# dark-Stallion/alac

Measured on AMD Instinct MI355X. Metric: encode Msamples/s (bit-exact) 44.1kHz/16-bit stereo, 1/2/4/8 GPU, higher is better.
Workload: dtype int32 (int16 PCM, int16 coefficients)

## Files before the change

### alac_amd/csrc/alac_encode_v1_impl.hpp

```cpp
#pragma once
#include <cstdlib>
#include <type_traits>
#include "alac_encode_v1_types.hpp"
#include "alac_lms.hpp"
#include "alac_golomb.hpp"

namespace alacdev {

template <int N, int I = 0, class F>
__device__ __forceinline__ void static_for(F &&f)
{
    if constexpr (I < N) {
        f(std::integral_constant<int, I>{});
        static_for<N, I + 1>(f);
    }
}

constexpr int kHist = 12;
template <int LPC>
struct Geo {
    static constexpr int TILE = LPC == 1 ? 32 : 64;
    static constexpr int ROWLEN = kHist + TILE;
    static constexpr int STRIDE = ROWLEN + 9;
};
// ... 266 lines not shown
        P.xs[it] = row * Geo<LPC>::STRIDE + kHist + grp * 4;
        const int32_t r = CH == 2 ? sh.rowMix[row] : 0;
        P.wl[it] = r ? r : (1 << kMixBits);
        P.wr[it] = r ? (1 << kMixBits) - r : 0;
        P.vsel[it] = r ? -1 : 0;
    }
}

template <int DEPTH, int CH, int LPC>
__device__ __forceinline__ void stage_load_fast(StageRegs<CH, LPC> &R, const StagePlan<CH, LPC> &P, int j0)
{
    constexpr int BPF = CH * (int)bytes_per_sample(DEPTH);
    const int64_t byteOff = (int64_t)j0 * BPF;
#pragma unroll
    for (int it = 0; it < StagePlan<CH, LPC>::ITERS; it++) task_load<DEPTH, CH>(P.pk[it] + byteOff, R.v[it]);
}

template <int LPC, bool HEAD = false>
__device__ __forceinline__ void keep_history(LmsShared<LPC> &sh, int lane)
{
    constexpr int SLOTS = 64 / LPC, N = kHist * SLOTS / 64;
    static_assert(kHist * SLOTS % 64 == 0, "every lane moves the same number of cells");
    int32_t v[N];
#pragma unroll
    for (int it = 0; it < N; it++) {
        const int idx = it * 64 + lane, row = idx % SLOTS, c = idx / SLOTS;
        v[it] = HEAD ? 0 : sh.xs[row * Geo<LPC>::STRIDE + Geo<LPC>::TILE + c];
    }
#pragma unroll
    for (int it = 0; it < N; it++) {
        const int idx = it * 64 + lane, row = idx % SLOTS, c = idx / SLOTS;
        sh.xs[row * Geo<LPC>::STRIDE + c] = v[it];
    }
}

template <int DEPTH, int CH, int LPC>
__device__ __forceinline__ void stage_store_fast(const StageRegs<CH, LPC> &R, const StagePlan<CH, LPC> &P,
                                                 LmsShared<LPC> &sh)
{
#pragma unroll
    for (int it = 0; it < StagePlan<CH, LPC>::ITERS; it++) {
        static_for<4>([&](auto T) {
            constexpr int t = decltype(T)::value;
            if constexpr (CH == 2) {
                const int32_t l = task_sample<DEPTH, 2 * t>(R.v[it]), r = task_sample<DEPTH, 2 * t + 1>(R.v[it]);
                sh.xs[P.xs[it] + t] = (__mul24(P.wl[it], l) + __mul24(P.wr[it], r)) >> kMixBits;
                sh.xs[P.xs[it] + Geo<LPC>::STRIDE + t] = P.vsel[it] ? l - r : r;
            } else {
                sh.xs[P.xs[it] + t] = task_sample<DEPTH, t>(R.v[it]);
            }
        });
    }
}

struct StepOps {
    int32_t nx[8], tp[8], cu[8];
};

__device__ __forceinline__ void load_ops(StepOps &o, const int32_t *pn, const int32_t *pt, const int32_t *pc)
{
#pragma unroll
    for (int s = 0; s < 8; s++) {
        o.nx[s] = pn[s];
        o.tp[s] = pt[s];
        o.cu[s] = pc[s];
    }
}

template <int T, int LPC, bool MASKED, bool DEAD = (T > 4)>
__device__ __forceinline__ void run_block(int32_t (&a)[T], int32_t (&w)[T], const StepOps &o, const LmsLaneT<T> &L, int jb,
                                          int32_t *resAt, uint32_t chanbits)
{
#pragma unroll
    for (int s = 0; s < 8; s++) {
        const int j = jb + s;
        const int32_t liveMask = MASKED ? (((j >= L.jlo) & (j < L.jhi)) ? -1 : 0) : -1;
        resAt[s] = lms_step<T, LPC, MASKED, DEAD>(a, w, o.tp[s], o.cu[s], liveMask, L, chanbits);
#pragma unroll
        for (int i = T - 1; i > 0; i--) w[i] = w[i - 1];
        w[0] = o.nx[s];
    }
}

struct LaneView {
    const int32_t *row;
    int32_t *res;
    const int32_t *zero;
    bool feeds;
};

template <int T, int LPC, bool DEAD = (T > 4)>
__device__ __forceinline__ void run_tile(int32_t (&a)[T], const LaneView &V, const LmsLaneT<T> &L, int j0, int jEnd,
                                         uint32_t chanbits)
{
    const int adv = V.feeds ? 1 : 0;
    const int32_t *pn = V.feeds ? V.row + kHist - T * L.h : V.zero;
    const int32_t *pt = V.feeds ? V.row + kHist - 1 - L.na : V.zero;
    const int32_t *pc = V.row + kHist;
    int32_t w[T];
#pragma unroll
    for (int i = 0; i < T; i++) w[i] = V.feeds ? V.row[kHist - 1 - T * L.h - i] : 0;
    StepOps opA, opB;
    load_ops(opA, pn, pt, pc);
    auto block = [&](const StepOps &cur, StepOps &nxt, int jb) {
        const int o = jb - j0;
        load_ops(nxt, pn + adv * (o + 8), pt + adv * (o + 8), pc + (o + 8));
        const bool allLive = __all((jb >= L.jlo) & (jb + 8 <= L.jhi));
        if (allLive)
            run_block<T, LPC, false, DEAD>(a, w, cur, L, jb, V.res + o, chanbits);
        else
            run_block<T, LPC, true, DEAD>(a, w, cur, L, jb, V.res + o, chanbits);
    };
    for (int jb = j0; jb < jEnd; jb += 16) {
        block(opA, opB, jb);
        if (jb + 8 < jEnd) block(opB, opA, jb + 8);
        else opA = opB;
    }
}

struct ChainJob {
    bool active;
    uint32_t seg, ch, p, N;
    int na;
    int16_t *row;
};

struct NoSink {};
template <int DEPTH, int CH, int LPC, bool WT = false, bool ZZ = false, int T = 4, class Sink = NoSink, bool DEAD = (T > 4)>
__device__ __forceinline__ void lms_pass(LmsShared<LPC> &sh, const V1Args &A, const ChainJob &J, int32_t (&a)[T],
                                         uint32_t num, uint32_t P, bool store, int32_t *dst, uint64_t streamStride,
                                         uint32_t stream, int lane, uint32_t *flag = nullptr, uint32_t flagBase = 0,
                                         StageRegs<CH, LPC> *head = nullptr, int headMode = 0, Sink *sink = nullptr)
{
    constexpr int SLOTS = 64 / LPC;
    constexpr uint32_t chanBits = DEPTH - 8 * bytes_shifted(DEPTH) + (CH == 2 ? 1 : 0);
    const uint32_t frameBytes = A.S.frameSize * CH * bytes_per_sample(DEPTH);
    const int slot = lane / LPC;
    LmsLaneT<T> L = make_lane<T, LPC>(lane, J.na, J.active ? (int)num : 0);
    const uint32_t idleVal = A.idleFast ? 0xffffffffu : 0u;
    if (!J.active && A.idleFast) {
        L.jlo = 0;
        L.jhi = 0x7fffffff;
    }
    LaneView V;
    V.feeds = J.active && (T * L.h < J.na);
    V.row = sh.xs + slot * Geo<LPC>::STRIDE;
    V.res = V.feeds ? sh.xs + slot * Geo<LPC>::STRIDE : sh.xs + SLOTS * Geo<LPC>::STRIDE;
    V.zero = sh.zero;
    const int fs = lane % SLOTS;
    const uint32_t fP = (uint32_t)__shfl((int)(J.active ? P : 0), fs * LPC);
    const uint32_t fStream = (uint32_t)__shfl((int)stream, fs * LPC);
    const int fNa = __shfl(J.na, fs * LPC);
    const uint32_t runTo = wave_max(J.active ? (store ? (P > num ? P : num) : num) : 0);
    const uint32_t half = (uint32_t)(lane / SLOTS);
    const uint32_t voff = half * (uint32_t)streamStride + fStream;
    const bool fAct = __shfl((int)J.active, fs * LPC) != 0;
    const uint32_t fPmin = wave_min_u32(fAct ? fP : idleVal);
    StageRegs<CH, LPC> R;
    StagePlan<CH, LPC> SP;
    stage_plan<DEPTH, CH, LPC>(SP, sh, A.S.pcm, frameBytes, lane);
    const uint32_t nMinRows = wave_min_u32(J.active ? J.N : idleVal);
    auto interior = [&](int j) { return SP.usable && (uint32_t)(j + Geo<LPC>::TILE) <= nMinRows; };
    if (runTo > 0) {
        if (interior(0)) {
            keep_history<LPC, true>(sh, lane);
            if (head && headMode == 2) {
                stage_store_fast<DEPTH, CH, LPC>(*head, SP, sh);
            } else {
                stage_load_fast<DEPTH, CH, LPC>(R, SP, 0);
                if (head && headMode == 1) {
                    constexpr int BPF = CH * (int)bytes_per_sample(DEPTH);
#pragma unroll
                    for (int it = 0; it < StagePlan<CH, LPC>::ITERS; it++)
#pragma unroll
                        for (int k = 0; k <= BPF; k++) head->v[it][k] = R.v[it][k];
                }
                stage_store_fast<DEPTH, CH, LPC>(R, SP, sh);
            }
        } else {
            stage_load<DEPTH, CH, LPC>(R, sh, A.S.pcm, frameBytes, 0, lane);
            stage_store<DEPTH, CH, LPC>(R, sh, A.S.pcm, frameBytes, 0, lane);
        }
    }
    for (int j0 = 0; j0 < (int)runTo; j0 += Geo<LPC>::TILE) {
        const bool more = j0 + Geo<LPC>::TILE < (int)runTo;
        const bool fastNext = more && interior(j0 + Geo<LPC>::TILE);
        if (fastNext) stage_load_fast<DEPTH, CH, LPC>(R, SP, j0 + Geo<LPC>::TILE);
        else if (more) stage_load<DEPTH, CH, LPC>(R, sh, A.S.pcm, frameBytes, j0 + Geo<LPC>::TILE, lane);
        lds_order();
        if (store && j0 == 0) {
            for (int pos = lane / SLOTS; pos <= fNa; pos += LPC) {
                const int32_t *xr = sh.xs + fs * Geo<LPC>::STRIDE + kHist;
                sh.xs[fs * Geo<LPC>::STRIDE + Geo<LPC>::ROWLEN + pos] = pos == 0 ? xr[0] : sext(xr[pos] - xr[pos - 1], 32 - chanBits);
            }
            lds_order();
        }
        const int jEnd = min(j0 + Geo<LPC>::TILE, (int)((runTo + 7) & ~7u));
        run_tile<T, LPC, DEAD>(a, V, L, j0, jEnd, chanBits);
        lds_order();
        if (store) {
            if (j0 == 0) {
                for (int pos = lane / SLOTS; pos <= fNa; pos += LPC)
                    sh.xs[fs * Geo<LPC>::STRIDE + pos] = sh.xs[fs * Geo<LPC>::STRIDE + Geo<LPC>::ROWLEN + pos];
                lds_order();
            }
            using Cell = int32_t __attribute__((ext_vector_type(4)));
            auto put4 = [&](const char *rowBase, uint32_t off, const int32_t *v) {
                auto zz = [](int32_t x) { return ZZ ? (int32_t)(((uint32_t)x << 1) ^ (uint32_t)(x >> 31)) : x; };
                Cell c;
                c.x = zz(v[0]);
                c.y = zz(v[1]);
                c.z = zz(v[2]);
                c.w = zz(v[3]);
                if constexpr (WT)
                    asm volatile("global_store_dwordx4 %0, %1, %2 sc1\n\ts_nop 1" : : "v"(off), "v"(c), "s"(rowBase) : "memory");
                else
                    *(Cell *)(rowBase + off) = c;
            };
            if constexpr (!std::is_same<Sink, NoSink>::value) {
                static_assert(LPC == 1, "a tile sink reads the lane's own row");
                (*sink)(j0, sh.xs + fs * Geo<LPC>::STRIDE);
            }
            constexpr int CELLS = Geo<LPC>::TILE / 4 / LPC;
            const int32_t *cell = sh.xs + fs * Geo<LPC>::STRIDE + 4 * (int)half;
            const char *rowPtr = dst ? (const char *)(dst + (uint64_t)j0 * streamStride) : nullptr;
            const uint64_t rowStep = (uint64_t)LPC * streamStride * 16u;
            const uint32_t laneOff = voff * 16u;
            if (!std::is_same<Sink, NoSink>::value && !dst) {
            } else if constexpr (LPC >= 2) {
                if ((uint32_t)(j0 + Geo<LPC>::TILE) <= fPmin) {
                    int32_t v[CELLS][4];
#pragma unroll
                    for (int it = 0; it < CELLS; it++)
#pragma unroll
                        for (int k = 0; k < 4; k++) v[it][k] = cell[it * 4 * LPC + k];
                    lds_order();
                    uint32_t off = laneOff;
                    asm volatile("" : "+v"(off));
#pragma unroll
                    for (int it = 0; it < CELLS; it++) {
                        put4(rowPtr, off, v[it]);
                        rowPtr += rowStep;
                    }
                } else {
                    constexpr int GROUP = 2;
                    static_assert(CELLS % GROUP == 0, "whole groups");
#pragma unroll 1
                    for (int g = 0; g < CELLS; g += GROUP) {
                        int32_t v[GROUP][4];
#pragma unroll
                        for (int k = 0; k < GROUP; k++)
#pragma unroll
                            for (int e = 0; e < 4; e++) v[k][e] = cell[(g + k) * 4 * LPC + e];
                        lds_order();
#pragma unroll
                        for (int k = 0; k < GROUP; k++) {
                            const uint32_t j = (uint32_t)(j0 + 4 * ((g + k) * LPC + (int)half));
                            if (j < fP) put4(rowPtr, laneOff, v[k]);
                            rowPtr += rowStep;
                        }
                        lds_order();
                    }
                }
            } else {
                const bool whole = (uint32_t)(j0 + Geo<LPC>::TILE) <= fPmin;
#pragma unroll
                for (int it = 0; it < CELLS; it++) {
                    int32_t v[4];
#pragma unroll
                    for (int k = 0; k < 4; k++) v[k] = cell[it * 4 + k];
                    if (whole || (uint32_t)(j0 + 4 * it) < fP) put4(rowPtr, laneOff, v);
                    rowPtr += rowStep;
                }
            }
            if (flag) {
                const uint32_t pm = A.pubMask & 0xffu;
                const uint32_t tile = (uint32_t)j0 / (uint32_t)Geo<LPC>::TILE;
                if ((tile & pm) == pm || (uint32_t)j0 + (pm + 1) * (uint32_t)Geo<LPC>::TILE >= runTo)
                    publish_rows(flag, flagBase + (uint32_t)min(j0 + Geo<LPC>::TILE, (int)runTo), lane, (A.pubMask >> 31) != 0, A.ho.lose);
            }
        }
// ... 3 lines not shown
            lds_order();
            stage_store_fast<DEPTH, CH, LPC>(R, SP, sh);
        } else if (more) {
            stage_store<DEPTH, CH, LPC>(R, sh, A.S.pcm, frameBytes, j0 + Geo<LPC>::TILE, lane);
        }
    }
}

template <int LPC>
__device__ __forceinline__ void lms_setup(LmsShared<LPC> &sh, const ChainJob &J, int mix, int lane)
{
    constexpr int SLOTS = 64 / LPC;
    if (lane < kZeroCells) sh.zero[lane] = 0;
    if (lane % LPC == 0) {
        const int slot = lane / LPC;
        sh.pktIdx[slot] = J.p;
        sh.pktN[slot] = J.active ? J.N : 0;
        sh.rowMix[slot] = mix;
    }
    (void)SLOTS;
    lds_order();
}

template <int LPC, int T = 4>
__device__ __forceinline__ void load_row(const ChainJob &J, int32_t (&a)[T], int lane, bool virgin = false)
{
    const int h = lane & (LPC - 1);
#pragma unroll
    for (int i = 0; i < T; i++) {
        const int k = T * h + i;
        const int32_t init = k == 0 ? 1216 : (k == 1 ? -928 : (k == 2 ? -64 : 0));
        a[i] = (J.active && k < J.na) ? (virgin ? init : (int32_t)J.row[k]) : 0;
    }
}

__device__ __forceinline__ int pick_mixres(const V1Args &A, uint32_t seg)
{
    uint32_t best = 0, minb = 1u << 31;
#pragma unroll
    for (uint32_t r = 0; r <= (uint32_t)kMaxRes; r++) {
        const uint32_t tot = A.bits1[r * A.chainsPad + seg * 2] + A.bits1[r * A.chainsPad + seg * 2 + 1];
        if (tot < minb) {
            minb = tot;
            best = r;
        }
    }
    return (int)best;
}

struct PacketDecision {
    uint32_t num[2];
    uint32_t escape;
};
template <int DEPTH, int CH>
__device__ __forceinline__ PacketDecision decide_packet(const V1Args &A, uint32_t seg, uint32_t N)
{
    constexpr uint32_t SHB = bytes_shifted(DEPTH);
    PacketDecision D;
    D.num[1] = 0;
    uint32_t minBits = 0;
#pragma unroll
    for (uint32_t c = 0; c < (uint32_t)CH; c++) {
        const uint32_t chain = seg * CH + c;
        const uint32_t c4 = A.cost2[chain], c8 = A.cost2[A.chainsPad + chain];
        D.num[c] = c8 < c4 ? 8 : 4;
        minBits += c8 < c4 ? c8 : c4;
    }
    const uint32_t partial = (N != A.S.frameSize);
    minBits += (CH == 2 ? 64 : 32) + (partial ? 32 : 0) + N * (SHB * 8) * CH;
    const uint32_t escapeBits = N * DEPTH * CH + (partial ? 32 : 0) + 16;
    D.escape = minBits >= escapeBits ? 1u : 0u;
    return D;
}

template <int LPC, int T = 4>
__device__ __forceinline__ void store_row(const ChainJob &J, const int32_t (&a)[T], int lane)
{
    const int h = lane & (LPC - 1);
#pragma unroll
    for (int i = 0; i < T; i++)
        if (J.active && T * h + i < J.na) J.row[T * h + i] = (int16_t)a[i];
}

template <int DEPTH, int T, int L>
__device__ __forceinline__ void search1_predictor(LmsShared<L> &sh, const V1Args &A, uint32_t block, int lane, uint32_t *flag)
{
    constexpr int SLOTS = 64 / L;
    ChainJob J;
    const uint32_t chain = A.S.segBegin * 2 + block * SLOTS + lane / L;
    J.seg = chain >> 1;
    J.ch = chain & 1;
    J.active = seg_packet(A.S, J.seg, J.p, J.N);
    J.na = 8;
    J.row = A.state + (uint64_t)J.seg * 64 + J.ch * 32 + 16;
    if (A.rowReady && A.S.pos > 0) {
        bool wait = false;
        if (J.active) {
            const PacketRec *prev = A.recs + (J.p - 1);
            wait = !prev->escape && prev->c[J.ch].num == 8;
        }
        bool seen = false;
        for (uint32_t spins = 0; spins < A.ho.spinLimit; spins++) {
            const uint32_t r = wait ? __hip_atomic_load(A.rowReady + chain, __ATOMIC_RELAXED, __HIP_MEMORY_SCOPE_AGENT) : 0xffffffffu;
            if (__all(r >= A.S.pos)) {
                seen = true;
                break;
            }
            __builtin_amdgcn_s_sleep(16);
        }
        if (!seen && A.ho.err && lane == 0) __hip_atomic_store(A.ho.err, 1u, __ATOMIC_RELAXED, __HIP_MEMORY_SCOPE_SYSTEM);
        __builtin_amdgcn_fence(__ATOMIC_ACQUIRE, "agent");
    }
    int32_t a[T];
    load_row<L>(J, a, lane, A.virgin != 0);
    const uint32_t n8 = J.N / 8;
    constexpr bool keepHead = L != 1;
    StageRegs<2, L> headRegs;
    StageRegs<2, L> *head = keepHead ? &headRegs : nullptr;
    for (int r = 0; r <= kMaxRes; r++) {
        lms_setup<L>(sh, J, r, lane);
        if (flag)
            lms_pass<DEPTH, 2, L, true>(sh, A, J, a, n8, n8, true, A.resA, 5ull * A.chainsPad, (uint32_t)r * A.chainsPad + chain,
                                        lane, flag, (uint32_t)r << 16, head, r == 0 ? 1 : 2);
        else
            lms_pass<DEPTH, 2, L>(sh, A, J, a, n8, n8, true, A.resA, 5ull * A.chainsPad, (uint32_t)r * A.chainsPad + chain, lane,
                                  nullptr, 0, head, r == 0 ? 1 : 2);
    }
    store_row<L>(J, a, lane);
    if (flag) publish_rows(flag, 0xffffffffu, lane, (A.pubMask >> 31) != 0, A.ho.lose);
}

template <int DEPTH, int T, int L>
__global__ __launch_bounds__(64, L == 1 ? 2 : 1) void k_lms_search1(V1Args A)
{
    __shared__ LmsShared<L> sh;
    search1_predictor<DEPTH, T, L>(sh, A, blockIdx.x, threadIdx.x, nullptr);
}

template <int DEPTH, int CH, int RS, int T, int LPC>
__device__ __forceinline__ void search2_body(LmsShared<LPC> &sh, const V1Args &A, uint32_t block, int lane)
{
    constexpr int SLOTS = 64 / LPC;
    constexpr int rs = RS;
    ChainJob J;
    const uint32_t chain = A.S.segBegin * CH + block * SLOTS + lane / LPC;
    J.seg = chain / CH;
    J.ch = chain % CH;
    J.active = seg_packet(A.S, J.seg, J.p, J.N);
    J.na = rs ? 8 : 4;
    J.row = A.state + (uint64_t)J.seg * 64 + J.ch * 32 + rs * 16;
    int32_t a[T];
    load_row<LPC>(J, a, lane, A.virgin != 0 && (rs == 0 || CH == 1));
    const int best = (CH == 2 && J.active) ? pick_mixres(A, J.seg) : 0;
    if (CH == 2 && rs == 1 && J.active && J.ch == 0 && (lane % LPC) == 0) A.recs[J.p].mixRes = (uint32_t)best;
    lms_setup<LPC>(sh, J, best, lane);
    const uint32_t n8 = J.N / 8, n32 = J.N / 32;
    StageRegs<CH, LPC> head;
    for (int pass = 0; pass < 8; pass++) {
        const bool last = pass == 7;
        const uint32_t num = (CH == 1 && last) ? n8 : n32;
        uint32_t P = num > (uint32_t)(J.na + 1) ? num : (uint32_t)(J.na + 1);
        P = P < n8 ? P : n8;
        lms_pass<DEPTH, CH, LPC>(sh, A, J, a, num, P, last, A.resB, 2ull * A.chainsPad, (uint32_t)rs * A.chainsPad + chain,
                                 lane, nullptr, 0, &head, pass == 0 ? 1 : 2);
    }
    store_row<LPC>(J, a, lane);
}

template <int DEPTH, int CH, int T3 = 4, int L3 = 1, int T7 = 4, int L7 = 2, int WAVES = 1>
__global__ __launch_bounds__(64, WAVES) void k_lms_search2(V1Args A, uint32_t nb3)
{
    __shared__ union {
        LmsShared<L3> s1;
        LmsShared<L7> s2;
    } sh;
    if (blockIdx.x < nb3)
        search2_body<DEPTH, CH, 0, T3, L3>(sh.s1, A, blockIdx.x, threadIdx.x);
    else
        search2_body<DEPTH, CH, 1, T7, L7>(sh.s2, A, blockIdx.x - nb3, threadIdx.x);
}

template <int DEPTH, int CH>
__global__ __launch_bounds__(64 * kWavesPerWg, 1) void k_lms_search2_w(V1Args A, uint32_t nb3, uint32_t nb7)
{
    __shared__ union {
        LmsShared<1> s1;
        LmsShared<2> s2;
    } shAll[kWavesPerWg];
    const Worker W = worker_id();
    auto &sh = shAll[W.slot];
    const uint32_t t = W.id / 3, r = W.id % 3;
    if (r == 0) {
        if (t < nb3) search2_body<DEPTH, CH, 0, 4, 1>(sh.s1, A, t, W.lane);
    } else {
        const uint32_t b = 2 * t + r - 1;
        if (b < nb7) search2_body<DEPTH, CH, 1, 4, 2>(sh.s2, A, b, W.lane);
    }
}

template <int DEPTH, int CH>
__global__ __launch_bounds__(64) void k_lms_final(V1Args A)
{
    __shared__ LmsShared<2> sh;
    const int lane = threadIdx.x;
    ChainJob J;
    const uint32_t chain = A.S.segBegin * CH + blockIdx.x * 32u + lane / 2;
    J.seg = chain / CH;
    J.ch = chain % CH;
    J.active = seg_packet(A.S, J.seg, J.p, J.N);
    J.na = 4;
    int best = 0;
    uint32_t N = J.N;
    if (J.active) {
        const PacketRec *rec = A.recs + J.p;
        J.na = rec->c[J.ch].num;
        best = (int)rec->mixRes;
        if (rec->escape) {
            J.active = false;
        }
    }
    J.row = A.state + (uint64_t)J.seg * 64 + J.ch * 32 + (J.na == 8 ? 16 : 0);
    int32_t a[4];
    load_row<2>(J, a, lane);
    lms_setup<2>(sh, J, best, lane);
    lms_pass<DEPTH, CH, 2, false, true>(sh, A, J, a, N, N, true, A.resC, A.chainsPad, chain, lane);
    store_row<2>(J, a, lane);
}


template <int CH>
__global__ __launch_bounds__(64) void k_gol_count1(V1Args A, uint32_t chanBits)
{
    __shared__ uint32_t recip[17];
    gol_table_init(recip, threadIdx.x);
    __syncthreads();
    const uint32_t chain = A.S.segBegin * CH + blockIdx.x * 64u + threadIdx.x, r = blockIdx.y;
    const uint32_t t = r * A.chainsPad + chain;
    uint32_t p, N;
    const bool active = seg_packet(A.S, chain / CH, p, N);
    const uint32_t n8 = active ? N / 8 : 0;
    const int32_t *plane = plane_from_stream(A.resA, (uint64_t)r * A.chainsPad);
    const uint64_t stride = 5ull * A.chainsPad;
    GolF g;
    golf_reset(g);
    golf_stream<false>(g, n8, wave_max(n8), chanBits, recip, one_plane(plane, stride, chain));
    if (active) A.bits1[t] = n8 ? g.bits : 0u;
}

template <int DEPTH, int T, int L, bool WALK = false>
__global__ __launch_bounds__(64 * kWavesPerWg, 1) void k_search1_fused(V1Args A, uint32_t nLms, uint32_t cblocks, uint32_t chanBits)
{
    __shared__ LmsShared<L> shAll[kWavesPerWg];
    __shared__ uint32_t recipAll[kWavesPerWg][20];
    const Worker W = worker_id();
    LmsShared<L> &sh = shAll[W.slot];
    uint32_t *recip = recipAll[W.slot];
    const int lane = W.lane;
    if constexpr (WALK) {
        if (W.id >= (uint32_t)(L + 1) * cblocks) return;
        const uint32_t t = W.id / (L + 1), r0 = W.id % (L + 1);
        if (r0 < (uint32_t)L) {
            const uint32_t pw = (uint32_t)L * t + r0;
            if (pw < nLms) search1_predictor<DEPTH, T, L>(sh, A, pw, lane, A.flags + pw);
            return;
        }
        gol_table_init(recip, lane);
        lds_order();
        const uint32_t w = t;
        const uint32_t chain = A.S.segBegin * 2 + w * 64u + lane;
        uint32_t p, N;
        const bool active = seg_packet(A.S, chain >> 1, p, N);
        const uint32_t n8 = active ? N / 8 : 0;
        const uint64_t stride = 5ull * A.chainsPad;
        RowWait wait;
        wait.producers(A.flags, L * w, L, nLms);
        wait.avail = 0;
        wait.ho = A.ho;
        const uint32_t nMax = wave_max(n8);
#pragma unroll 1
        for (uint32_t r = 0; r <= (uint32_t)kMaxRes; r++) {
            GolF g;
            golf_reset(g);
            wait.base = r << 16;
            golf_stream<false>(g, n8, nMax, chanBits, recip, one_plane(plane_from_stream(A.resA, (uint64_t)r * A.chainsPad), stride, chain), wait);
            if (active) A.bits1[r * A.chainsPad + chain] = n8 ? g.bits : 0u;
        }
        return;
    }
    if (W.id >= nLms + 5 * cblocks) return;
    if (W.id < nLms) {
        search1_predictor<DEPTH, T, L>(sh, A, W.id, lane, A.flags + W.id);
    } else {
        gol_table_init(recip, lane);
        lds_order();
        const uint32_t idx = W.id - nLms, r = idx / cblocks, w = idx % cblocks;
        const uint32_t chain = A.S.segBegin * 2 + w * 64u + lane;
        const uint32_t t = r * A.chainsPad + chain;
        uint32_t p, N;
        const bool active = seg_packet(A.S, chain >> 1, p, N);
        const uint32_t n8 = active ? N / 8 : 0;
        const int32_t *plane = plane_from_stream(A.resA, (uint64_t)r * A.chainsPad);
        const uint64_t stride = 5ull * A.chainsPad;
        GolF g;
        golf_reset(g);
        RowWait wait;
        wait.producers(A.flags, L * w, L, nLms);
        wait.avail = 0;
        wait.base = r << 16;
        wait.ho = A.ho;
        golf_stream<false>(g, n8, wave_max(n8), chanBits, recip, one_plane(plane, stride, chain), wait);
        if (active) A.bits1[t] = n8 ? g.bits : 0u;
    }
}

template <int CH, class Need>
__device__ __forceinline__ void count2_body(const V1Args &A, uint32_t chain, uint32_t rs, uint32_t chanBits, const uint32_t *recip,
                                            Need &&need)
{
    const uint32_t t = rs * A.chainsPad + chain;
    uint32_t p, N;
    const bool active = seg_packet(A.S, chain / CH, p, N);
    const uint32_t n8 = active ? N / 8 : 0, n32 = N / 32, na = rs ? 8 : 4;
    uint32_t P2 = n8;
    if (CH == 2) {
        P2 = n32 > na + 1 ? n32 : na + 1;
        P2 = P2 < n8 ? P2 : n8;
    }
    const uint64_t strideB = 2ull * A.chainsPad, strideA = 5ull * A.chainsPad;
    GolF g;
    golf_reset(g);
    const int32_t *planeB = plane_from_stream(A.resB, (uint64_t)rs * A.chainsPad), *planeA = plane_from_stream(A.resA, (uint64_t)kMaxRes * A.chainsPad);
    const uint32_t nMax = wave_max(n8);
    const uint32_t p2lo = wave_min_u32(active ? P2 : 0xffffffffu), p2hi = wave_max(active ? P2 : 0u);
    if (CH == 1 || p2lo >= p2hi) {
        RowSrc rs2;
        rs2.p0 = planeB;
        rs2.s0 = strideB;
        rs2.p1 = planeA;
        rs2.s1 = strideA;
        rs2.split = CH == 1 ? 0xffffffffu : p2hi;
        rs2.col = chain;
        rs2.org = 0;
        golf_stream<false>(g, n8, nMax, chanBits, recip, rs2, need);
    } else {
        golf_stream_fn<false>(g, n8, nMax, chanBits, recip, [&](uint32_t j) {
            const int32_t b = planeB[plane_index(j, strideB, chain)], a = planeA[plane_index(j, strideA, chain)];
            return j < P2 ? b : a;
        }, need);
    }
    if (active) A.cost2[t] = (n8 ? g.bits : 0u) * 8 + 16 * na;
}

template <int CH>
__global__ __launch_bounds__(64) void k_gol_count2(V1Args A, uint32_t chanBits)
{
    __shared__ uint32_t recip[17];
    gol_table_init(recip, threadIdx.x);
    __syncthreads();
    count2_body<CH>(A, A.S.segBegin * CH + blockIdx.x * 64u + threadIdx.x, blockIdx.y, chanBits, recip, NoWait());
}

template <int CH>
__global__ __launch_bounds__(64 * kWavesPerWg, 1) void k_gol_count2_w(V1Args A, uint32_t cblocks, uint32_t chanBits)
{
    __shared__ uint32_t recipAll[kWavesPerWg][20];
    const Worker W = worker_id();
    if (W.id >= 2 * cblocks) return;
    uint32_t *recip = recipAll[W.slot];
    gol_table_init(recip, W.lane);
    lds_order();
    count2_body<CH>(A, A.S.segBegin * CH + (W.id % cblocks) * 64u + (uint32_t)W.lane, W.id / cblocks, chanBits, recip, NoWait());
}

#ifdef ALAC_V1_COMMON_TU
// ... 78 lines not shown
    __shared__ LmsShared<L> shAll[kWavesPerWg];
    __shared__ uint32_t recipAll[kWavesPerWg][20];
    const Worker W = worker_id();
    if (W.id >= nWorkers) return;
    LmsShared<L> &sh = shAll[W.slot];
    uint32_t *recip = recipAll[W.slot];
    const int lane = W.lane;
    uint32_t wid = W.id;
    if constexpr (!SPLIT) {
        const uint32_t t = W.id / (L + 1), r = W.id % (L + 1);
        wid = r < (uint32_t)L ? (uint32_t)L * t + r : nLms + t;
        if (r < (uint32_t)L && wid >= nLms) return;
    }
    struct WaveStamp {
        uint32_t *p;
        __device__ __forceinline__ WaveStamp(uint32_t *dbg, int lane) : p(dbg ? dbg + 8ull * (blockIdx.x * (uint32_t)kWavesPerWg + (threadIdx.x >> 6)) : nullptr)
        {
            if (p && lane == 0) {
                const uint64_t t = __builtin_amdgcn_s_memtime();
                p[0] = __builtin_amdgcn_s_getreg((31 << 11) | 4);
                p[1] = __builtin_amdgcn_s_getreg((31 << 11) | 20);
                p[2] = (uint32_t)t;
                p[3] = (uint32_t)(t >> 32);
            }
        }
        __device__ __forceinline__ void done(int lane)
        {
            if (p && lane == 0) {
                const uint64_t t = __builtin_amdgcn_s_memtime();
                p[4] = (uint32_t)t;
                p[5] = (uint32_t)(t >> 32);
                p[6] = __builtin_amdgcn_s_getreg((31 << 11) | 4);
            }
        }
    } stamp(A.dbg, lane);
    if (wid < nLms) {
        ChainJob J;
        const uint32_t chain = A.S.segBegin * CH + wid * (64u / L) + lane / L;
        J.seg = chain / CH;
        J.ch = chain % CH;
        J.active = seg_packet(A.S, J.seg, J.p, J.N);
        J.na = 4;
        int best = 0;
        const uint32_t N = J.N;
        const bool have = J.active;
        if (J.active) {
            if constexpr (FOLD) {
                const PacketDecision D = decide_packet<DEPTH, CH>(A, J.seg, N);
                J.na = (int)D.num[J.ch];
                best = CH == 2 ? (int)A.recs[J.p].mixRes : 0;
                if (D.escape) J.active = false;
            } else {
                const PacketRec *rec = A.recs + J.p;
                J.na = rec->c[J.ch].num;
                best = (int)rec->mixRes;
                if (rec->escape) J.active = false;
            }
        }
        J.row = A.state + (uint64_t)J.seg * 64 + J.ch * 32 + (J.na == 8 ? 16 : 0);
        int32_t a[T];
        load_row<L>(J, a, lane);
        if constexpr (FOLD) {
            if (have) {
                PacketRec *rec = A.recs + J.p;
                const int h = lane & (L - 1);
#pragma unroll
                for (int i = 0; i < T; i++)
                    if (T * h + i < 8) rec->c[J.ch].coefs[T * h + i] = (T * h + i < J.na) ? (int16_t)a[i] : (int16_t)0;
                if (h == 0) {
                    rec->c[J.ch].num = (uint16_t)J.na;
                    if (J.ch == 0) {
                        rec->numSamples = N;
                        if (CH == 1) {
                            rec->c[1].num = 0;
                            rec->c[1].bits = 0;
                            rec->mixRes = 0;
                        }
                    }
                }
            }
        }
        lms_setup<L>(sh, J, best, lane);
        uint32_t *flag = A.flagsF + wid;
        lms_pass<DEPTH, CH, L, true, true>(sh, A, J, a, N, N, true, A.resC, A.chainsPad, chain, lane, flag);
        store_row<L>(J, a, lane);
        if (A.rowReady) {
            asm volatile("s_waitcnt vmcnt(0)" ::: "memory");
            __builtin_amdgcn_fence(__ATOMIC_RELEASE, "agent");
            asm volatile("s_waitcnt vmcnt(0)" ::: "memory");
            if (J.active && J.na == 8 && lane % L == 0 && !A.ho.lose)
                __hip_atomic_store(A.rowReady + chain, A.S.pos + 1, __ATOMIC_RELAXED, __HIP_MEMORY_SCOPE_AGENT);
        }
        publish_rows(flag, 0xffffffffu, lane, (A.pubMask >> 31) != 0, A.ho.lose);
        stamp.done(lane);
    } else {
        gol_table_init(recip, lane);
        lds_order();
        const uint32_t cb = wid - nLms;
        const bool second = SPLIT && cb >= nCoder;
        const uint32_t w = second ? cb - nCoder : cb;
        const uint32_t chain = A.S.segBegin * CH + w * 64u + lane;
        uint32_t p, N;
        bool active = seg_packet(A.S, chain / CH, p, N);
        const bool have = active;
        PacketRec *rec = A.recs + p;
        PacketDecision D;
        D.num[0] = D.num[1] = D.escape = 0;
        if constexpr (FOLD) {
            if (have) D = decide_packet<DEPTH, CH>(A, chain / CH, N);
            if (D.escape) active = false;
        } else {
            if (active && rec->escape) active = false;
        }
        const uint32_t c = chain % CH;
        const uint32_t n = active ? N : 0;
        const int32_t *plane = A.resC;
        const uint64_t stride = A.chainsPad;
        GolF g;
        golf_reset(g);
        const uint64_t slotIdx = have ? (uint64_t)p * 2 + c : (uint64_t)A.dumpSlot + c;
        RowWait wait;
        wait.producers(A.flagsF, L * w, L, nLms);
        wait.avail = 0;
        wait.base = 0;
        wait.ho = A.ho;
        if constexpr (!SPLIT) {
            uint32_t *slot = A.bitWords + slotIdx * A.wcap;
            golf_open(g, slot, A.wcap);
            golf_stream<true, true, RowWait &, LAZY>(g, n, wave_max(n), chanBits, recip, one_plane(plane, stride, chain), wait,
                                                     A.idleFast != 0);
            golf_flush<true, LAZY>(g);
            const uint32_t bits = active ? golf_written_bits<LAZY>(g, slot) : 0u;
            if (active) rec->c[c].bits = bits;
            if constexpr (FOLD) {
                const uint32_t other = CH == 2 ? (uint32_t)__shfl_xor((int)bits, 1) : 0u;
                if (have && c == 0) {
                    constexpr uint32_t SHB = bytes_shifted(DEPTH);
                    const uint32_t partial = (N != A.S.frameSize);
                    const uint32_t escapeBits = N * DEPTH * CH + (partial ? 32 : 0) + 16;
                    bool esc = D.escape != 0;
                    uint32_t body = 0;
                    if (!esc) {
                        body = 12 + 4 + (partial ? 32 : 0) + 16 + N * (SHB * 8) * CH + (16 + 16 * D.num[0] + bits);
                        if (CH == 2) body += 16 + 16 * D.num[1] + other;
                        if (body >= escapeBits) esc = true;
                    }
                    if (esc) body = 12 + 4 + (partial ? 32 : 0) + N * DEPTH * CH;
                    rec->escape = esc ? 1u : 0u;
                    rec->totalBits = 7 + body + 3;
                    A.packetBytes[p] = (7 + body + 3 + 7) / 8;
                }
            }
        } else {
            const uint32_t a = A.splitAt;
            const uint32_t nA = min(n, a), nB = n - nA;
            if (!second) {
                uint32_t *slot = A.bitWords + slotIdx * A.wcap;
                golf_open(g, slot, A.wcap);
                golf_stream<true, true>(g, nA, wave_max(nA), chanBits, recip, one_plane(plane, stride, chain), wait,
                                        A.idleFast != 0, n <= a);
                golf_flush<true>(g);
                if (active) rec->c[c].bits = golf_written_bits(g, slot);
            } else {
                golf_stream<false, true>(g, nA, wave_max(nA), chanBits, recip, one_plane(plane, stride, chain), wait,
                                         A.idleFast != 0, false);
                g.bits = 0;
                uint32_t *slot = A.bitWordsB + slotIdx * A.wcap;
// ... 498 lines not shown
```

### alac_amd/csrc/alac_lms.hpp

```cpp
#pragma once

#include <stdint.h>
#if defined(__HIPCC__)
#include "alac_dev.hpp"
#define ALAC_RULE_FN __device__ __forceinline__
#else
#include <algorithm>
#define ALAC_RULE_FN inline
#endif

namespace alacdev {

#if defined(__HIPCC__)
constexpr int kDppXor1 = 0xB1;

__device__ __forceinline__ int32_t dpp_xor1(int32_t src)
{
    return __builtin_amdgcn_update_dpp(0, src, kDppXor1, 0xf, 0xf, true);
}

__device__ __forceinline__ int32_t med3_i32(int32_t x, int32_t lo, int32_t hi)
{
    int32_t r;
    asm("v_med3_i32 %0, %1, %2, %3" : "=v"(r) : "v"(x), "v"(lo), "v"(hi));
// ... 48 lines not shown
    return __builtin_amdgcn_update_dpp(0, src, CTRL, 0xf, 0xf, true);
}

template <int T>
struct LmsLaneT {
    int32_t h;
    int32_t na;
    int32_t wg[T];
    int32_t act[T];
    int32_t c255;
    int32_t carry1;
    int32_t carry2;
    int32_t jlo, jhi;
};

template <int T, int L>
__device__ __forceinline__ LmsLaneT<T> make_lane(int lane, int na, int num)
{
    LmsLaneT<T> R;
    R.h = L == 1 ? 0 : (lane & (L - 1));
    R.na = na;
#pragma unroll
    for (int i = 0; i < T; i++) {
        const int kk = T * R.h + i;
        R.wg[i] = kk < na ? na - kk : 0;
        R.act[i] = kk < na ? -1 : 0;
    }
    R.c255 = R.h == 0 ? 255 : 0;
    R.carry1 = (R.h + 1 < L) ? -1 : 0;
    R.carry2 = (R.h + 2 < L) ? -1 : 0;
    R.jlo = na + 1;
    R.jhi = num;
    return R;
}

template <int T, int L, bool MASKED, bool DEAD = (T > 4)>
__device__ __forceinline__ int32_t lms_step(int32_t (&a)[T], const int32_t (&w)[T], int32_t tp, int32_t cu,
                                            int32_t liveMask, const LmsLaneT<T> &R, uint32_t chanbits)
{
    int32_t b[T];
#pragma unroll
    for (int i = 0; i < T; i++) b[i] = tp - w[i];
    const int32_t p = cu - tp;
    int32_t s = R.c255;
#pragma unroll
    for (int i = 0; i < T; i++) s = __mul24((int32_t)(int16_t)a[i], b[i]) + s;
    if constexpr (L >= 2) s += dpp_xor1(s);
    if constexpr (L == 4) s += dpp_quad<kDppXor2>(s);
    const int32_t del = __builtin_amdgcn_sbfe(p + (s >> kDenShift), 0, chanbits);

    const int32_t nd = -del;
    const int32_t adel = max(del, nd);
    int32_t nsg = sign3(nd);
    if constexpr (MASKED) nsg &= liveMask;
    const int32_t rc = (del >> 31) & ((1 << kDenShift) - 1);
    int32_t sb[T];
    uint32_t t[T];
#pragma unroll
    for (int i = 0; i < T; i++) {
        sb[i] = sign3(b[i]);
        if constexpr (DEAD) sb[i] &= R.act[i];
        t[i] = (uint32_t)(__mul24(sb[i], b[i]) + rc) >> kDenShift;
    }
    int32_t S[T];
    S[T - 1] = 0;
#pragma unroll
    for (int i = T - 1; i > 0; i--) S[i - 1] = (int32_t)__umul24(t[i], (uint32_t)R.wg[i]) + S[i];
    int32_t adj = adel;
    if constexpr (L >= 2) {
        const int32_t tot = (int32_t)__umul24(t[0], (uint32_t)R.wg[0]) + S[0];
        if constexpr (L == 2) {
            adj = adel - (dpp_xor1(tot) & R.carry1);
        } else {
            const int32_t up1 = dpp_quad<kDppShl1>(tot) & R.carry1;
            const int32_t pair = tot + up1;
            adj = adel - up1 - (dpp_quad<kDppShl2>(pair) & R.carry2);
        }
    }
#pragma unroll
    for (int i = 0; i < T; i++) a[i] = __mul24(adj > S[i] ? nsg : 0, sb[i]) + a[i];
    return del;
}

using LmsLane = LmsLaneT<4>;
template <int LPC, bool MASKED>
__device__ __forceinline__ int32_t lms4_step(int32_t (&a)[4], const int32_t (&w)[4], int32_t tp, int32_t cu,
                                             int32_t liveMask, const LmsLane &R, uint32_t chanbits)
{
    return lms_step<4, LPC, MASKED>(a, w, tp, cu, liveMask, R, chanbits);
}

struct LmsDecLane {
    int32_t h;
    int32_t wg[4];
    int32_t c255, carryMask;
    int32_t topMine;
    int32_t takeOut;
    int32_t feed;
};

__device__ __forceinline__ LmsDecLane make_dec_lane(int lane, int na)
{
    LmsDecLane L;
    L.h = lane & 1;
#pragma unroll
    for (int i = 0; i < 4; i++) {
        const int kk = 4 * L.h + i;
        L.wg[i] = kk < na ? na - kk : 0;
    }
    L.c255 = L.h == 0 ? 255 : 0;
    L.carryMask = L.h == 0 ? -1 : 0;
    L.topMine = (L.h == (na == 8 ? 1 : 0)) ? -1 : 0;
    L.takeOut = L.h == 0 ? -1 : 0;
    L.feed = (L.h == 0 || na == 8) ? -1 : 0;
    return L;
}

__device__ __forceinline__ int32_t lms4_step_dec(int32_t (&a)[4], int32_t (&w)[4], int32_t &tp, int32_t del,
                                                 const LmsDecLane &L, uint32_t chanbits)
{
    int32_t b[4];
#pragma unroll
    for (int i = 0; i < 4; i++) b[i] = tp - w[i];
    int32_t s = L.c255;
#pragma unroll
    for (int i = 0; i < 4; i++) s = __mul24((int32_t)(int16_t)a[i], b[i]) + s;
    s += dpp_xor1(s);
    const int32_t out = __builtin_amdgcn_sbfe(del + tp - (s >> kDenShift), 0, chanbits);

    const int32_t nd = -del;
    const int32_t adel = max(del, nd);
    const int32_t nsg = sign3(nd);
    const int32_t rc = (del >> 31) & ((1 << kDenShift) - 1);
    int32_t sb[4];
    uint32_t t[4];
#pragma unroll
    for (int i = 0; i < 4; i++) {
        sb[i] = sign3(b[i]);
        t[i] = (uint32_t)(__mul24(sb[i], b[i]) + rc) >> kDenShift;
    }
    int32_t S[4];
    S[3] = 0;
#pragma unroll
    for (int i = 3; i > 0; i--) S[i - 1] = (int32_t)__umul24(t[i], (uint32_t)L.wg[i]) + S[i];
    const int32_t tot = (int32_t)__umul24(t[0], (uint32_t)L.wg[0]) + S[0];
    const int32_t adj = adel - (dpp_xor1(tot) & L.carryMask);
#pragma unroll
    for (int i = 0; i < 4; i++) a[i] = __mul24(adj > S[i] ? nsg : 0, sb[i]) + a[i];
    const int32_t x = dpp_xor1(w[3]) & L.feed;
    tp = L.topMine ? w[3] : x;
    w[3] = w[2];
    w[2] = w[1];
    w[1] = w[0];
    w[0] = L.takeOut ? out : x;
    return out;
}

#endif

}

#undef ALAC_RULE_FN
```

Baseline: 29950.

## Add hand-scheduled lone-wave LMS step with software-pipelined operand prep

Adds an LMS step variant for 4-tap LPC=1/2 chains that precomputes the next step's differences, signs and partial dot products, and interleaves that work into the current step's serial dependency chain. Scheduling barriers and asm pins fix the instruction order. The point is to hide ALU latency on the recursive update path when few waves are resident. The variant is enabled in search2, in search1 for L=2, and in the final pass. It raises register pressure and makes the code depend on a fixed instruction order that can fight the compiler.

```diff
diff --git a/alac_amd/csrc/alac_encode_v1_impl.hpp b/alac_amd/csrc/alac_encode_v1_impl.hpp
--- a/alac_amd/csrc/alac_encode_v1_impl.hpp
+++ b/alac_amd/csrc/alac_encode_v1_impl.hpp
@@ -372,6 +372,72 @@
     }
 }
 
+struct StepPrep {
+    int32_t b[8][4], sb[8][4], p[8];
+};
+
+__device__ __forceinline__ void prep_sub(StepPrep &P, const StepOps &o, const int32_t (&w0)[4], int t, int m)
+{
+    if (m < 4) P.b[t][m] = o.tp[t] - (m < t ? o.nx[m < t ? t - 1 - m : 0] : w0[m < t ? 0 : m - t]);
+    else P.p[t] = o.cu[t] - o.tp[t];
+}
+
+struct LoneFill {
+    StepOps &co, &no;
+    StepPrep &cur, &nxt;
+    const int32_t (&w0)[4];
+    int s;
+    int m = 0, i = 0;
+    __device__ __forceinline__ void sub(int n)
+    {
+        const int32_t none[4] = {0, 0, 0, 0};
+        StepOps &o = s == 0 ? co : no;
+        StepPrep &P = s == 0 ? cur : nxt;
+        const int t = s == 0 ? 7 : s - 1;
+#pragma unroll
+        for (int r = 0; r < n; r++, m++) {
+            if (m > 4) break;
+            prep_sub(P, o, s == 0 ? none : w0, t, m);
+            if (m < 4) ALAC_PIN(P.b[t][m]);
+            else ALAC_PIN(P.p[t]);
+        }
+        if (m <= 4) ALAC_ARM(o.tp[t]);
+        else if (s < 7) ALAC_ARM(no.tp[s]);
+    }
+    __device__ __forceinline__ void sgn()
+    {
+        StepPrep &P = s < 2 ? cur : nxt;
+        const int t = s < 2 ? 6 + s : s - 2;
+        if (i < 4) P.sb[t][i] = sign3_pinned(P.b[t][i]);
+        i++;
+    }
+};
+
+template <int LPC, bool MASKED>
+__device__ __forceinline__ void run_block_lone(int32_t (&a)[4], LoneCarry &C, StepOps &co, StepPrep &cur, StepOps &no, StepPrep &nxt,
+                                               const int32_t (&w0)[4], const LmsLaneT<4> &L, int jb, int32_t *resAt, uint32_t chanbits)
+{
+    int32_t dPrev = 0;
+#pragma unroll
+    for (int s = 0; s < 8; s++) {
+        const int j = jb + s;
+        const int32_t liveMask = MASKED ? (((j >= L.jlo) & (j < L.jhi)) ? -1 : 0) : -1;
+        LoneFill fill{co, no, cur, nxt, w0, s};
+        const int32_t del = s < 7 ? lms_step_lone<LPC, MASKED>(a, C, cur.b[s], cur.sb[s], cur.p[s], cur.b[s < 7 ? s + 1 : 7], liveMask, L, chanbits, fill)
+                                  : lms_step_lone<LPC, MASKED>(a, C, cur.b[s], cur.sb[s], cur.p[s], nxt.b[0], liveMask, L, chanbits, fill);
+        fill.sub(5);
+#pragma unroll
+        for (int r = 0; r < 4; r++) fill.sgn();
+        if (s & 1) {
+            resAt[s - 1] = dPrev;
+            resAt[s] = del;
+            __builtin_amdgcn_sched_barrier(0);
+        } else {
+            dPrev = del;
+        }
+    }
+}
+
 struct LaneView {
     const int32_t *row;
     int32_t *res;
@@ -379,7 +445,7 @@
     bool feeds;
 };
 
-template <int T, int LPC, bool DEAD = (T > 4)>
+template <int T, int LPC, bool DEAD = (T > 4), bool LONE = false>
 __device__ __forceinline__ void run_tile(int32_t (&a)[T], const LaneView &V, const LmsLaneT<T> &L, int j0, int jEnd,
                                          uint32_t chanbits)
 {
@@ -392,6 +458,37 @@
     for (int i = 0; i < T; i++) w[i] = V.feeds ? V.row[kHist - 1 - T * L.h - i] : 0;
     StepOps opA, opB;
     load_ops(opA, pn, pt, pc);
+    if constexpr (LONE) {
+        static_assert(T == 4 && !DEAD && LPC <= 2, "the lone-wave step is built for <4, 1> and <4, 2>");
+        StepPrep pA, pB;
+#pragma unroll
+        for (int t = 0; t < 7; t++) {
+#pragma unroll
+            for (int m = 0; m < 5; m++) prep_sub(pA, opA, w, t, m);
+#pragma unroll
+            for (int i = 0; i < 4; i++)
+                if (t < 6) pA.sb[t][i] = sign3(pA.b[t][i]);
+        }
+        LoneCarry C;
+        lone_products(C, a, pA.b[0], L);
+        auto block = [&](StepOps &curOps, StepPrep &cur, StepOps &nxtOps, StepPrep &nxt, int jb) {
+            const int o = jb - j0;
+            load_ops(nxtOps, pn + adv * (o + 8), pt + adv * (o + 8), pc + (o + 8));
+            int32_t w0[4];
+#pragma unroll
+            for (int i = 0; i < 4; i++) w0[i] = curOps.nx[7 - i];
+            const bool allLive = __all((jb >= L.jlo) & (jb + 8 <= L.jhi));
+            if (allLive)
+                run_block_lone<LPC, false>(a, C, curOps, cur, nxtOps, nxt, w0, L, jb, V.res + o, chanbits);
+            else
+                run_block_lone<LPC, true>(a, C, curOps, cur, nxtOps, nxt, w0, L, jb, V.res + o, chanbits);
+        };
+        for (int jb = j0; jb < jEnd; jb += 16) {
+            block(opA, pA, opB, pB, jb);
+            if (jb + 8 < jEnd) block(opB, pB, opA, pA, jb + 8);
+        }
+        return;
+    }
     auto block = [&](const StepOps &cur, StepOps &nxt, int jb) {
         const int o = jb - j0;
         load_ops(nxt, pn + adv * (o + 8), pt + adv * (o + 8), pc + (o + 8));
@@ -416,7 +513,7 @@
 };
 
 struct NoSink {};
-template <int DEPTH, int CH, int LPC, bool WT = false, bool ZZ = false, int T = 4, class Sink = NoSink, bool DEAD = (T > 4)>
+template <int DEPTH, int CH, int LPC, bool WT = false, bool ZZ = false, int T = 4, class Sink = NoSink, bool DEAD = (T > 4), bool LONE = false>
 __device__ __forceinline__ void lms_pass(LmsShared<LPC> &sh, const V1Args &A, const ChainJob &J, int32_t (&a)[T],
                                          uint32_t num, uint32_t P, bool store, int32_t *dst, uint64_t streamStride,
                                          uint32_t stream, int lane, uint32_t *flag = nullptr, uint32_t flagBase = 0,
@@ -486,7 +583,7 @@
             lds_order();
         }
         const int jEnd = min(j0 + Geo<LPC>::TILE, (int)((runTo + 7) & ~7u));
-        run_tile<T, LPC, DEAD>(a, V, L, j0, jEnd, chanBits);
+        run_tile<T, LPC, DEAD, LONE>(a, V, L, j0, jEnd, chanBits);
         lds_order();
         if (store) {
             if (j0 == 0) {
@@ -656,7 +753,7 @@
         if (J.active && T * h + i < J.na) J.row[T * h + i] = (int16_t)a[i];
 }
 
-template <int DEPTH, int T, int L>
+template <int DEPTH, int T, int L, bool LONE = false>
 __device__ __forceinline__ void search1_predictor(LmsShared<L> &sh, const V1Args &A, uint32_t block, int lane, uint32_t *flag)
 {
     constexpr int SLOTS = 64 / L;
@@ -694,7 +791,7 @@
     for (int r = 0; r <= kMaxRes; r++) {
         lms_setup<L>(sh, J, r, lane);
         if (flag)
-            lms_pass<DEPTH, 2, L, true>(sh, A, J, a, n8, n8, true, A.resA, 5ull * A.chainsPad, (uint32_t)r * A.chainsPad + chain,
+            lms_pass<DEPTH, 2, L, true, false, T, NoSink, (T > 4), LONE>(sh, A, J, a, n8, n8, true, A.resA, 5ull * A.chainsPad, (uint32_t)r * A.chainsPad + chain,
                                         lane, flag, (uint32_t)r << 16, head, r == 0 ? 1 : 2);
         else
             lms_pass<DEPTH, 2, L>(sh, A, J, a, n8, n8, true, A.resA, 5ull * A.chainsPad, (uint32_t)r * A.chainsPad + chain, lane,
@@ -711,7 +808,7 @@
     search1_predictor<DEPTH, T, L>(sh, A, blockIdx.x, threadIdx.x, nullptr);
 }
 
-template <int DEPTH, int CH, int RS, int T, int LPC>
+template <int DEPTH, int CH, int RS, int T, int LPC, bool LONE = false>
 __device__ __forceinline__ void search2_body(LmsShared<LPC> &sh, const V1Args &A, uint32_t block, int lane)
 {
     constexpr int SLOTS = 64 / LPC;
@@ -735,7 +832,7 @@
         const uint32_t num = (CH == 1 && last) ? n8 : n32;
         uint32_t P = num > (uint32_t)(J.na + 1) ? num : (uint32_t)(J.na + 1);
         P = P < n8 ? P : n8;
-        lms_pass<DEPTH, CH, LPC>(sh, A, J, a, num, P, last, A.resB, 2ull * A.chainsPad, (uint32_t)rs * A.chainsPad + chain,
+        lms_pass<DEPTH, CH, LPC, false, false, T, NoSink, (T > 4), LONE>(sh, A, J, a, num, P, last, A.resB, 2ull * A.chainsPad, (uint32_t)rs * A.chainsPad + chain,
                                  lane, nullptr, 0, &head, pass == 0 ? 1 : 2);
     }
     store_row<LPC>(J, a, lane);
@@ -765,10 +862,10 @@
     auto &sh = shAll[W.slot];
     const uint32_t t = W.id / 3, r = W.id % 3;
     if (r == 0) {
-        if (t < nb3) search2_body<DEPTH, CH, 0, 4, 1>(sh.s1, A, t, W.lane);
+        if (t < nb3) search2_body<DEPTH, CH, 0, 4, 1, true>(sh.s1, A, t, W.lane);
     } else {
         const uint32_t b = 2 * t + r - 1;
-        if (b < nb7) search2_body<DEPTH, CH, 1, 4, 2>(sh.s2, A, b, W.lane);
+        if (b < nb7) search2_body<DEPTH, CH, 1, 4, 2, true>(sh.s2, A, b, W.lane);
     }
 }
 
@@ -835,7 +932,7 @@
         const uint32_t t = W.id / (L + 1), r0 = W.id % (L + 1);
         if (r0 < (uint32_t)L) {
             const uint32_t pw = (uint32_t)L * t + r0;
-            if (pw < nLms) search1_predictor<DEPTH, T, L>(sh, A, pw, lane, A.flags + pw);
+            if (pw < nLms) search1_predictor<DEPTH, T, L, (T == 4 && L == 2)>(sh, A, pw, lane, A.flags + pw);
             return;
         }
         gol_table_init(recip, lane);
@@ -863,7 +960,7 @@
     }
     if (W.id >= nLms + 5 * cblocks) return;
     if (W.id < nLms) {
-        search1_predictor<DEPTH, T, L>(sh, A, W.id, lane, A.flags + W.id);
+        search1_predictor<DEPTH, T, L, (T == 4 && L == 2)>(sh, A, W.id, lane, A.flags + W.id);
     } else {
         gol_table_init(recip, lane);
         lds_order();
@@ -1108,7 +1205,7 @@
         }
         lms_setup<L>(sh, J, best, lane);
         uint32_t *flag = A.flagsF + wid;
-        lms_pass<DEPTH, CH, L, true, true>(sh, A, J, a, N, N, true, A.resC, A.chainsPad, chain, lane, flag);
+        lms_pass<DEPTH, CH, L, true, true, T, NoSink, (T > 4), (T == 4 && L == 2)>(sh, A, J, a, N, N, true, A.resC, A.chainsPad, chain, lane, flag);
         store_row<L>(J, a, lane);
         if (A.rowReady) {
             asm volatile("s_waitcnt vmcnt(0)" ::: "memory");
diff --git a/alac_amd/csrc/alac_lms.hpp b/alac_amd/csrc/alac_lms.hpp
--- a/alac_amd/csrc/alac_lms.hpp
+++ b/alac_amd/csrc/alac_lms.hpp
@@ -154,6 +154,149 @@
     return del;
 }
 
+struct LoneCarry {
+    int32_t s1, m1, m0;
+};
+
+#define ALAC_PIN(x)                          \
+    do {                                     \
+        asm volatile("" : : "v"(x));         \
+        __builtin_amdgcn_sched_barrier(0);   \
+    } while (0)
+#define ALAC_ARM(x) asm volatile("" : "+v"(x))
+
+__device__ __forceinline__ int32_t sign3_pinned(int32_t x)
+{
+    int32_t r;
+    asm volatile("v_med3_i32 %0, %1, -1, 1" : "=v"(r) : "v"(x));
+    __builtin_amdgcn_sched_barrier(0);
+    return r;
+}
+
+__device__ __forceinline__ void lone_products(LoneCarry &C, const int32_t (&a)[4], const int32_t (&bn)[4], const LmsLaneT<4> &R)
+{
+    C.s1 = __mul24((int32_t)(int16_t)a[3], bn[3]) + __mul24((int32_t)(int16_t)a[2], bn[2]) + R.c255;
+    C.m1 = __mul24((int32_t)(int16_t)a[1], bn[1]);
+    C.m0 = __mul24((int32_t)(int16_t)a[0], bn[0]);
+}
+
+template <int L, bool MASKED, class Fill>
+__device__ __forceinline__ int32_t lms_step_lone(int32_t (&a)[4], LoneCarry &C, const int32_t (&b)[4], const int32_t (&sb)[4],
+                                                 int32_t p, const int32_t (&bn)[4], int32_t liveMask, const LmsLaneT<4> &R,
+                                                 uint32_t chanbits, Fill &&fill)
+{
+    static_assert(L == 1 || L == 2, "the lone-wave mappings");
+    constexpr int32_t kRc = (1 << kDenShift) - 1;
+    int32_t s = C.s1 + C.m1 + C.m0;
+    ALAC_PIN(s);
+    if constexpr (L == 2) {
+        fill.sub(2);
+        s += dpp_xor1(s);
+        ALAC_PIN(s);
+    }
+    fill.sgn();
+    s >>= kDenShift;
+    ALAC_PIN(s);
+    fill.sgn();
+    s += p;
+    ALAC_PIN(s);
+    fill.sgn();
+    int32_t del = __builtin_amdgcn_sbfe(s, 0, chanbits);
+    ALAC_PIN(del);
+    fill.sgn();
+    int32_t nd = -del;
+    ALAC_PIN(nd);
+    int32_t rc = del >> 31;
+    ALAC_PIN(rc);
+    int32_t adel = max(del, nd);
+    ALAC_PIN(adel);
+    rc &= kRc;
+    ALAC_PIN(rc);
+    int32_t nsg = sign3_pinned(nd);
+    if constexpr (MASKED) {
+        nsg &= liveMask;
+        ALAC_PIN(nsg);
+    }
+    int32_t u3 = __mul24(sb[3], b[3]) + rc;
+    ALAC_PIN(u3);
+    int32_t u2 = __mul24(sb[2], b[2]) + rc;
+    ALAC_PIN(u2);
+    int32_t t3 = (int32_t)((uint32_t)u3 >> kDenShift);
+    ALAC_PIN(t3);
+    int32_t u1 = __mul24(sb[1], b[1]) + rc;
+    ALAC_PIN(u1);
+    int32_t t2 = (int32_t)((uint32_t)u2 >> kDenShift);
+    ALAC_PIN(t2);
+    int32_t S2 = (int32_t)__umul24((uint32_t)t3, (uint32_t)R.wg[3]);
+    ALAC_PIN(S2);
+    int32_t u0 = 0;
+    if constexpr (L == 2) {
+        u0 = __mul24(sb[0], b[0]) + rc;
+        ALAC_PIN(u0);
+    }
+    int32_t t1 = (int32_t)((uint32_t)u1 >> kDenShift);
+    ALAC_PIN(t1);
+    int32_t S1 = (int32_t)__umul24((uint32_t)t2, (uint32_t)R.wg[2]) + S2;
+    ALAC_PIN(S1);
+    int32_t S0, adj;
+    if constexpr (L == 2) {
+        int32_t t0 = (int32_t)((uint32_t)u0 >> kDenShift);
+        ALAC_PIN(t0);
+        S0 = (int32_t)__umul24((uint32_t)t1, (uint32_t)R.wg[1]) + S1;
+        ALAC_PIN(S0);
+        fill.sub(1);
+        int32_t tot = (int32_t)__umul24((uint32_t)t0, (uint32_t)R.wg[0]) + S0;
+        ALAC_PIN(tot);
+        fill.sub(2);
+        int32_t up = dpp_xor1(tot) & R.carry1;
+        ALAC_PIN(up);
+        adj = adel - up;
+        ALAC_PIN(adj);
+    } else {
+        fill.sub(2);
+        S0 = (int32_t)__umul24((uint32_t)t1, (uint32_t)R.wg[1]) + S1;
+        ALAC_PIN(S0);
+        fill.sub(2);
+        adj = adel;
+    }
+    const bool c3 = adj > 0;
+    __builtin_amdgcn_sched_barrier(0);
+    const bool c2 = adj > S2;
+    __builtin_amdgcn_sched_barrier(0);
+    const bool c1 = adj > S1;
+    __builtin_amdgcn_sched_barrier(0);
+    const bool c0 = adj > S0;
+    __builtin_amdgcn_sched_barrier(0);
+    int32_t g3 = L == 1 ? nsg : (c3 ? nsg : 0);
+    if constexpr (L == 2) ALAC_PIN(g3);
+    int32_t g2 = c2 ? nsg : 0;
+    ALAC_PIN(g2);
+    a[3] = __mul24(g3, sb[3]) + a[3];
+    ALAC_PIN(a[3]);
+    int32_t g1 = c1 ? nsg : 0;
+    ALAC_PIN(g1);
+    a[2] = __mul24(g2, sb[2]) + a[2];
+    ALAC_PIN(a[2]);
+    int32_t n3 = __mul24((int32_t)(int16_t)a[3], bn[3]);
+    ALAC_PIN(n3);
+    int32_t g0 = c0 ? nsg : 0;
+    ALAC_PIN(g0);
+    a[1] = __mul24(g1, sb[1]) + a[1];
+    ALAC_PIN(a[1]);
+    int32_t n2 = __mul24((int32_t)(int16_t)a[2], bn[2]);
+    ALAC_PIN(n2);
+    a[0] = __mul24(g0, sb[0]) + a[0];
+    ALAC_PIN(a[0]);
+    C.m1 = __mul24((int32_t)(int16_t)a[1], bn[1]);
+    ALAC_PIN(C.m1);
+    C.s1 = n3 + n2 + R.c255;
+    ALAC_PIN(C.s1);
+    C.m0 = __mul24((int32_t)(int16_t)a[0], bn[0]);
+    ALAC_PIN(C.m0);
+    if constexpr (L == 1) fill.sub(1);
+    return del;
+}
+
 using LmsLane = LmsLaneT<4>;
 template <int LPC, bool MASKED>
 __device__ __forceinline__ int32_t lms4_step(int32_t (&a)[4], const int32_t (&w)[4], int32_t tp, int32_t cu,
```

Measured after the change: 30570, median of 6. 1.02x the previous value.
